# drprojects/DeepViewAgg

Measured on NVIDIA H100. Metric: Mpoints/s through view-agg fwd+bwd, higher is better.
Workload: dtype f32

## Files before the change

### deepviewagg_b200/csrc/view_attention.cuh

```cuda
#pragma once
#include "dva_common.cuh"

namespace dva {

struct VAParams {
  const void* x; const void* idx; int idx64;
  const float* compat; const int64_t* ptr;
  const float* gate_w; const float* gate_b;
  void* out; float* att; float* seg_max; float* seg_den; int32_t* seg_arg;
  const void* gout; const float* s_max; const float* s_den; const int32_t* s_arg;
  void* gx; float* gcompat; float* gate_partial; int scatter;
  int64_t N, V, R;
  int C, G, group_scaling;
  float eps;
};

constexpr int kTileStride = 33;

__device__ __forceinline__ float group_lane_sum(float v, int G) {
  for (int off = 16; off >= G; off >>= 1) v += __shfl_xor_sync(0xffffffffu, v, off);
  return v;
}

__device__ __forceinline__ uint32_t smem_u32(const void* p) { return (uint32_t)__cvta_generic_to_shared(p); }
__device__ __forceinline__ void mbar_init(uint32_t bar, uint32_t count) {
  asm volatile("mbarrier.init.shared::cta.b64 [%0], %1;" ::"r"(bar), "r"(count) : "memory");
}
__device__ __forceinline__ void mbar_init_fence() { asm volatile("fence.mbarrier_init.release.cluster;" ::: "memory"); }
__device__ __forceinline__ void mbar_expect_tx(uint32_t bar, uint32_t bytes) {
  asm volatile("mbarrier.arrive.expect_tx.shared::cta.b64 _, [%0], %1;" ::"r"(bar), "r"(bytes) : "memory");
}
__device__ __forceinline__ void mbar_wait(uint32_t bar, uint32_t parity) {
  uint32_t ok = 0;
  while (!ok) {
    asm volatile(
        "{ .reg .pred p; mbarrier.try_wait.parity.shared::cta.b64 p, [%1], %2; selp.u32 %0, 1, 0, p; }"
        : "=r"(ok) : "r"(bar), "r"(parity) : "memory");
  }
}
__device__ __forceinline__ void bulk_g2s(uint32_t dst, const void* src, uint32_t bytes, uint32_t bar) {
  asm volatile("cp.async.bulk.shared::cluster.global.mbarrier::complete_tx::bytes [%0], [%1], %2, [%3];"
               ::"r"(dst), "l"(src), "r"(bytes), "r"(bar) : "memory");
}
__device__ __forceinline__ void fence_proxy_async() { asm volatile("fence.proxy.async.shared::cta;" ::: "memory"); }

__device__ __forceinline__ uint32_t load_row_id(const void* idx, int idx64, int64_t v) {
  if (idx == nullptr) return (uint32_t)v;
  return idx64 ? (uint32_t) reinterpret_cast<const int64_t*>(idx)[v]
               : (uint32_t) reinterpret_cast<const int32_t*>(idx)[v];
}
__device__ __forceinline__ float sel4(const float4& v, int g) {
  return g == 0 ? v.x : (g == 1 ? v.y : (g == 2 ? v.z : v.w));
}

__device__ __forceinline__ float gate_t(float z) { return tanhf(fmaxf(z, 0.f)); }
__device__ __forceinline__ float4 gate_z4(const float4& w, const float4& m, const float4& b) {
  return make_float4(fmaf(w.x, m.x, b.x), fmaf(w.y, m.y, b.y), fmaf(w.z, m.z, b.z), fmaf(w.w, m.w, b.w));
}
__device__ __forceinline__ float4 gate_t4(const float4& z) {
  return make_float4(gate_t(z.x), gate_t(z.y), gate_t(z.z), gate_t(z.w));
}

__device__ __forceinline__ float gate_grad(float S, float z, float t, float w, float m, bool keep, float& dw,
                                           float& db) {
  if (!(z > 0.f)) return 0.f;
  const float dLdt = (t != 0.f) ? S / t : 0.f;
  const float u = dLdt * (1.f - t * t);
  const float dq = u * w;
  if (keep) {
    dw += u * m;
    db += u;
  }
  return dq;
}
__device__ __forceinline__ float4 gate_grad4(const float4& S, const float4& z, const float4& t, const float4& w,
                                             const float4& m, bool keep, float4& dw, float4& db) {
  return make_float4(gate_grad(S.x, z.x, t.x, w.x, m.x, keep, dw.x, db.x),
                     gate_grad(S.y, z.y, t.y, w.y, m.y, keep, dw.y, db.y),
                     gate_grad(S.z, z.z, t.z, w.z, m.z, keep, dw.z, db.z),
                     gate_grad(S.w, z.w, t.w, w.w, m.w, keep, dw.w, db.w));
}

__device__ __forceinline__ float compat_grad(float a, float sv, float S, float inv_sq, bool is_arg, float dq) {
  float d = a * (sv - S) * inv_sq;
  if (is_arg) d += dq;
  return d;
}
__device__ __forceinline__ float4 compat_grad4(const float4& a, const float4& sv, const float4& S, float inv_sq,
                                               int v, const int4& arg, const float4& dq) {
  return make_float4(compat_grad(a.x, sv.x, S.x, inv_sq, v == arg.x, dq.x),
                     compat_grad(a.y, sv.y, S.y, inv_sq, v == arg.y, dq.y),
                     compat_grad(a.z, sv.z, S.z, inv_sq, v == arg.z, dq.z),
                     compat_grad(a.w, sv.w, S.w, inv_sq, v == arg.w, dq.w));
}

template <int WARPS>
__device__ __forceinline__ void store_gate_partial(float* __restrict__ partial, const float4& dw, const float4& db) {
  __shared__ float gate_s[WARPS][8];
  const int warp = threadIdx.x >> 5, lane = threadIdx.x & 31;
  float v[8] = {dw.x, dw.y, dw.z, dw.w, db.x, db.y, db.z, db.w};
#pragma unroll
  for (int q = 0; q < 8; ++q) {
#pragma unroll
    for (int o = 16; o > 0; o >>= 1) v[q] += __shfl_xor_sync(0xffffffffu, v[q], o);
  }
  if (lane == 0) {
#pragma unroll
    for (int q = 0; q < 8; ++q) gate_s[warp][q] = v[q];
  }
  __syncthreads();
  if ((int)threadIdx.x < 8) {
    float acc = 0.f;
    for (int w = 0; w < WARPS; ++w) acc += gate_s[w][threadIdx.x];
    partial[(int64_t)blockIdx.x * 8 + threadIdx.x] = acc;
  }
}

template <typename K>
int range_geometry(K kern, size_t smem, int warps_per_cta, int max_ctas_per_sm, int ranges_per_warp, int64_t N,
                   const char* what, int* grid_out, int* pr_out) {
  cudaError_t e = cudaFuncSetAttribute(kern, cudaFuncAttributeMaxDynamicSharedMemorySize, (int)smem);
  if (e != cudaSuccess) return failf((int)e, "%s: %zu bytes of shared memory: %s", what, smem, cudaGetErrorString(e));
  int occ = 0;
  if (cudaOccupancyMaxActiveBlocksPerMultiprocessor(&occ, kern, warps_per_cta * 32, smem) != cudaSuccess || occ < 1) occ = 1;
  if (occ > max_ctas_per_sm) occ = max_ctas_per_sm;
  int64_t grid = (int64_t)kNumSMs * occ;
  const int64_t slots = grid * warps_per_cta * ranges_per_warp;
  int64_t pr = (N + slots - 1) / slots;
  if (pr < 8) pr = 8;
  const int64_t n_ranges = (N + pr - 1) / pr;
  const int64_t need = (n_ranges + warps_per_cta - 1) / warps_per_cta;
  if (grid > need) grid = need;
  if (grid < 1) grid = 1;
  *grid_out = (int)grid; *pr_out = (int)pr;
  return DVA_OK;
}

int va_ring_fwd(const VAParams& P, int dtype, cudaStream_t st);
int va_ring_bwd(const VAParams& P, int dtype, int* grid_out, cudaStream_t st);
int va_lane_bwd(const VAParams& P, int dtype, int* grid_out, cudaStream_t st);

}
```

### deepviewagg_b200/csrc/view_attention_lane.cu

```cuda
#include "view_attention.cuh"

namespace dva {

constexpr int kLaneWarps = 4;
constexpr uint32_t kFull = 0xffffffffu;

struct LaneSmem {
  float wt[32][4];
  float at[32][4];
  float st[32][4];
  float Sp[32][4];
  float dq[32][4];
  uint32_t ri[32];
  uint32_t orow[32];
  uint32_t go[32];
  uint64_t bar;
  uint64_t pad;
};

template <typename T, int LPR>
__global__ void __launch_bounds__(kLaneWarps * 32, 5)
va_lane_bwd_kernel(const VAParams P, const int PR) {
  constexpr int VEC = Vec16<T>::N, RPI = 32 / LPR, CPE = LPR / 4, U = 4, RS = LPR * 16;
  extern __shared__ __align__(128) unsigned char rows_all[];
  __shared__ LaneSmem sm_all[kLaneWarps];
  const int warp = threadIdx.x >> 5, lane = threadIdx.x & 31;
  LaneSmem& sm = sm_all[warp];
  unsigned char* rows_s = rows_all + (size_t)warp * 32 * RS;
  const uint32_t rows_u = smem_u32(rows_s), bar_u = smem_u32(&sm.bar);
  uint32_t uses = 0;
  if (lane == 0) {
    mbar_init(bar_u, 1);
    mbar_init_fence();
  }
  __syncwarp();
  const int sg = lane / LPR, lir = lane % LPR, gk = lir / CPE;
  const uint32_t row_bytes = (uint32_t)P.C * sizeof(T);
  const char* __restrict__ xbase = reinterpret_cast<const char*>(P.x);
  const char* __restrict__ gob = reinterpret_cast<const char*>(P.gout) + lir * 16;
  char* __restrict__ gxb = reinterpret_cast<char*>(P.gx) + lir * 16;
  const bool gating = P.gate_w != nullptr;
  float4 gw4 = make_float4(0.f, 0.f, 0.f, 0.f), gb4 = gw4;
  if (gating) {
    gw4 = make_float4(P.gate_w[0], P.gate_w[1], P.gate_w[2], P.gate_w[3]);
    gb4 = make_float4(P.gate_b[0], P.gate_b[1], P.gate_b[2], P.gate_b[3]);
  }
  float4 dw4 = make_float4(0.f, 0.f, 0.f, 0.f), db4 = dw4;
  const bool scatter = P.scatter && P.idx != nullptr;

  auto issue_rows = [&](int nv, uint32_t rid) {
    fence_proxy_async();
    __syncwarp();
    if (lane == 0) mbar_expect_tx(bar_u, (uint32_t)nv * row_bytes);
    __syncwarp();
    if (lane < nv) bulk_g2s(rows_u + (uint32_t)lane * RS, xbase + (uint64_t)rid * row_bytes, row_bytes, bar_u);
  };
  auto wait_rows = [&]() {
    mbar_wait(bar_u, uses & 1u);
    ++uses;
  };

  auto rows_phase = [&](int nv, int64_t pg) {
    for (int u0 = 0; u0 < nv; u0 += RPI * U) {
      uint4 xr[U], gr[U];
      float w[U];
      uint32_t orow[U];
      bool ok[U];
#pragma unroll
      for (int q = 0; q < U; ++q) {
        const int u = u0 + q * RPI + sg;
        ok[q] = u < nv;
        const int uu = ok[q] ? u : 0;
        orow[q] = sm.orow[uu];
        w[q] = sm.wt[uu][gk];
        xr[q] = *reinterpret_cast<const uint4*>(rows_s + (size_t)uu * RS + lir * 16);
        gr[q] = *reinterpret_cast<const uint4*>(gob + (uint64_t)(pg + sm.go[uu]) * row_bytes);
      }
#pragma unroll
      for (int q = 0; q < U; ++q) {
        float fx[VEC], fg[VEC], dx[VEC];
        unpack16<T, VEC>(xr[q], fx);
        unpack16<T, VEC>(gr[q], fg);
        float dot = 0.f;
#pragma unroll
        for (int j = 0; j < VEC; ++j) {
          dot = fmaf(fg[j], fx[j], dot);
          dx[j] = w[q] * fg[j];
        }
        if (ok[q]) stg_stream16(gxb + (uint64_t)orow[q] * row_bytes, pack16<T, VEC>(dx));
#pragma unroll
        for (int o = 1; o < CPE; o <<= 1) dot += __shfl_xor_sync(kFull, dot, o);
        if (ok[q] && (lir & (CPE - 1)) == 0) sm.st[u0 + q * RPI + sg][gk] = dot;
      }
    }
  };

  const int64_t n_ranges = (P.N + PR - 1) / PR;
  const int64_t warps_total = (int64_t)gridDim.x * kLaneWarps;
  for (int64_t r = (int64_t)blockIdx.x * kLaneWarps + warp; r < n_ranges; r += warps_total) {
    const int64_t pa = r * PR;
    const int64_t pb = (pa + PR < P.N) ? pa + PR : P.N;
    for (int64_t pg = pa; pg < pb;) {
      const int64_t pk = pg + lane;
      const bool valid = pk < pb;
      const int64_t p0 = valid ? P.ptr[pk] : 0;
      const int cnt = valid ? (int)(P.ptr[pk + 1] - p0) : 0;
      int incl = cnt;
#pragma unroll
      for (int o = 1; o < 32; o <<= 1) {
        const int t = __shfl_up_sync(kFull, incl, o);
        if (lane >= o) incl += t;
      }
      const int excl = incl - cnt;
      const unsigned fitm = __ballot_sync(kFull, valid && incl <= 32);
      const int kfit = (fitm == kFull) ? 32 : __ffs(~fitm) - 1;
      const int64_t gvb = __shfl_sync(kFull, p0, 0);

      if (kfit == 0) {
        const int n = __shfl_sync(kFull, cnt, 0);
        const float4 smx = reinterpret_cast<const float4*>(P.s_max)[pg];
        const float4 sdn = reinterpret_cast<const float4*>(P.s_den)[pg];
        const int4 sar = reinterpret_cast<const int4*>(P.s_arg)[pg];
        const float inv_sq = P.group_scaling ? rsqrtf((float)n) : 1.f;
        float4 z4 = make_float4(1.f, 1.f, 1.f, 1.f), t4 = z4;
        if (gating) {
          z4 = gate_z4(gw4, smx, gb4);
          t4 = gate_t4(z4);
        }
        float4 Sacc = make_float4(0.f, 0.f, 0.f, 0.f);
        for (int c0 = 0; c0 < n; c0 += 32) {
          const int nv = (n - c0 < 32) ? n - c0 : 32;
          const int64_t v = gvb + c0 + lane;
          float4 a = make_float4(0.f, 0.f, 0.f, 0.f);
          __syncwarp();
          const uint32_t rid_l = lane < nv ? load_row_id(P.idx, P.idx64, v) : 0u;
          issue_rows(nv, rid_l);
          if (lane < nv) {
            const float4 c = __ldg(reinterpret_cast<const float4*>(P.compat) + v);
            a = make_float4(__expf((c.x - smx.x) * inv_sq) / sdn.x, __expf((c.y - smx.y) * inv_sq) / sdn.y,
                            __expf((c.z - smx.z) * inv_sq) / sdn.z, __expf((c.w - smx.w) * inv_sq) / sdn.w);
            sm.ri[lane] = rid_l;
            sm.orow[lane] = scatter ? rid_l : (uint32_t)v;
            sm.go[lane] = 0u;
            *reinterpret_cast<float4*>(sm.wt[lane]) = make_float4(a.x * t4.x, a.y * t4.y, a.z * t4.z, a.w * t4.w);
          }
          __syncwarp();
          wait_rows();
          rows_phase(nv, pg);
          __syncwarp();
          if (lane < nv) {
            const float4 raw = *reinterpret_cast<const float4*>(sm.st[lane]);
            const float4 sp = make_float4(raw.x * t4.x, raw.y * t4.y, raw.z * t4.z, raw.w * t4.w);
            Sacc.x = fmaf(a.x, sp.x, Sacc.x); Sacc.y = fmaf(a.y, sp.y, Sacc.y);
            Sacc.z = fmaf(a.z, sp.z, Sacc.z); Sacc.w = fmaf(a.w, sp.w, Sacc.w);
            reinterpret_cast<float4*>(P.gcompat)[v] = sp;
          }
        }
#pragma unroll
        for (int o = 16; o > 0; o >>= 1) {
          Sacc.x += __shfl_xor_sync(kFull, Sacc.x, o); Sacc.y += __shfl_xor_sync(kFull, Sacc.y, o);
          Sacc.z += __shfl_xor_sync(kFull, Sacc.z, o); Sacc.w += __shfl_xor_sync(kFull, Sacc.w, o);
        }
        float4 dq = make_float4(0.f, 0.f, 0.f, 0.f);
        if (gating) dq = gate_grad4(Sacc, z4, t4, gw4, smx, lane == 0, dw4, db4);
        __syncwarp();
        for (int c0 = lane; c0 < n; c0 += 32) {
          const int64_t v = gvb + c0;
          const float4 c = __ldg(reinterpret_cast<const float4*>(P.compat) + v);
          const float4 sp = __ldcg(reinterpret_cast<const float4*>(P.gcompat) + v);
          float4 d;
          d.x = __expf((c.x - smx.x) * inv_sq) / sdn.x * (sp.x - Sacc.x) * inv_sq;
          d.y = __expf((c.y - smx.y) * inv_sq) / sdn.y * (sp.y - Sacc.y) * inv_sq;
          d.z = __expf((c.z - smx.z) * inv_sq) / sdn.z * (sp.z - Sacc.z) * inv_sq;
          d.w = __expf((c.w - smx.w) * inv_sq) / sdn.w * (sp.w - Sacc.w) * inv_sq;
          if ((int)v == sar.x) d.x += dq.x;
          if ((int)v == sar.y) d.y += dq.y;
          if ((int)v == sar.z) d.z += dq.z;
          if ((int)v == sar.w) d.w += dq.w;
          reinterpret_cast<float4*>(P.gcompat)[v] = d;
        }
        pg += 1;
        continue;
      }

      const int nv = __shfl_sync(kFull, incl, kfit - 1);
      int mp = 0;
      for (int k = 0; k < kfit; ++k) {
        const int s = __shfl_sync(kFull, excl, k), c = __shfl_sync(kFull, cnt, k);
        if (lane >= s && lane < s + c) mp = k;
      }
      const int cntp = __shfl_sync(kFull, cnt, mp);
      float4 a = make_float4(0.f, 0.f, 0.f, 0.f), t4 = make_float4(1.f, 1.f, 1.f, 1.f);
      float inv_sq = 1.f;
      int4 sar = make_int4(-1, -1, -1, -1);
      const int64_t v = gvb + lane;
      __syncwarp();
      const uint32_t rid_m = lane < nv ? load_row_id(P.idx, P.idx64, v) : 0u;
      if (nv > 0) issue_rows(nv, rid_m);
      if (lane < nv) {
        const float4 c = __ldg(reinterpret_cast<const float4*>(P.compat) + v);
        const float4 smx = reinterpret_cast<const float4*>(P.s_max)[pg + mp];
        const float4 sdn = reinterpret_cast<const float4*>(P.s_den)[pg + mp];
        sar = reinterpret_cast<const int4*>(P.s_arg)[pg + mp];
        inv_sq = P.group_scaling ? rsqrtf((float)cntp) : 1.f;
        a = make_float4(__expf((c.x - smx.x) * inv_sq) / sdn.x, __expf((c.y - smx.y) * inv_sq) / sdn.y,
                        __expf((c.z - smx.z) * inv_sq) / sdn.z, __expf((c.w - smx.w) * inv_sq) / sdn.w);
        if (gating) t4 = gate_t4(gate_z4(gw4, smx, gb4));
        sm.ri[lane] = rid_m;
        sm.orow[lane] = scatter ? rid_m : (uint32_t)v;
        sm.go[lane] = (uint32_t)mp;
        *reinterpret_cast<float4*>(sm.at[lane]) = a;
        *reinterpret_cast<float4*>(sm.wt[lane]) = make_float4(a.x * t4.x, a.y * t4.y, a.z * t4.z, a.w * t4.w);
      }
      __syncwarp();

      if (nv > 0) wait_rows();
      rows_phase(nv, pg);
      __syncwarp();

      if (lane < nv) {
        float4 raw = *reinterpret_cast<const float4*>(sm.st[lane]);
        raw.x *= t4.x; raw.y *= t4.y; raw.z *= t4.z; raw.w *= t4.w;
        *reinterpret_cast<float4*>(sm.st[lane]) = raw;
      }
      __syncwarp();
      if (lane < kfit) {
        float4 S = make_float4(0.f, 0.f, 0.f, 0.f), dq = S;
        for (int j = 0; j < cnt; ++j) {
          const float4 aa = *reinterpret_cast<const float4*>(sm.at[excl + j]);
          const float4 sv = *reinterpret_cast<const float4*>(sm.st[excl + j]);
          S.x = fmaf(aa.x, sv.x, S.x); S.y = fmaf(aa.y, sv.y, S.y); S.z = fmaf(aa.z, sv.z, S.z); S.w = fmaf(aa.w, sv.w, S.w);
        }
        if (gating && cnt > 0) {
          const float4 smx = reinterpret_cast<const float4*>(P.s_max)[pk];
          const float4 z4 = gate_z4(gw4, smx, gb4);
          dq = gate_grad4(S, z4, gate_t4(z4), gw4, smx, true, dw4, db4);
        }
        *reinterpret_cast<float4*>(sm.Sp[lane]) = S;
        *reinterpret_cast<float4*>(sm.dq[lane]) = dq;
      }
      __syncwarp();
      if (lane < nv) {
        const float4 S = *reinterpret_cast<const float4*>(sm.Sp[mp]);
        const float4 dq = *reinterpret_cast<const float4*>(sm.dq[mp]);
        const float4 sv = *reinterpret_cast<const float4*>(sm.st[lane]);
        reinterpret_cast<float4*>(P.gcompat)[v] = compat_grad4(a, sv, S, inv_sq, (int)v, sar, dq);
      }
      pg += kfit;
    }
  }

  if (P.gate_partial != nullptr) store_gate_partial<kLaneWarps>(P.gate_partial, dw4, db4);
}

int va_lane_bwd(const VAParams& P, int dtype, int* grid_out, cudaStream_t st) {
  return with_dtype(dtype, [&](auto tag) {
    using T = decltype(tag);
    return with_lpr(P.C / Vec16<T>::N, [&](auto lpr) {
      constexpr int LPR = decltype(lpr)::value;
      auto kern = va_lane_bwd_kernel<T, LPR>;
      const size_t smem = (size_t)kLaneWarps * 32 * LPR * 16;
      int grid, pr;
      if (int rc = range_geometry(kern, smem, kLaneWarps, 8, 4, P.N, "va_lane_bwd", &grid, &pr)) return rc;
      kern<<<grid, kLaneWarps * 32, smem, st>>>(P, pr);
      *grid_out = grid;
      return check_launch("va_lane_bwd");
    });
  });
}

}
```

Baseline: 54.22.

## Prefetch next point group rows and bulk-store dx in lane backward kernel

Restructures the lane backward kernel so that, for LPR==32, the next group's ptr ends and x rows are loaded ahead and issued via TMA while the current group finishes. dx rows are staged in shared memory and written back with a bulk async store using an evict_first L2 hint instead of per-thread streaming stores. Segment bookkeeping is simplified by loading cumulative ends directly instead of doing a prefix scan, and single-point groups use warp-shuffle reductions and a register-held gradient row instead of shared-memory round trips. The cost is more complex synchronization (bulk wait_group before reusing the row buffer) and lower min-blocks in the launch bounds for LPR==32.

```diff
diff --git a/deepviewagg_b200/csrc/view_attention.cuh b/deepviewagg_b200/csrc/view_attention.cuh
--- a/deepviewagg_b200/csrc/view_attention.cuh
+++ b/deepviewagg_b200/csrc/view_attention.cuh
@@ -43,6 +43,15 @@
                ::"r"(dst), "l"(src), "r"(bytes), "r"(bar) : "memory");
 }
 __device__ __forceinline__ void fence_proxy_async() { asm volatile("fence.proxy.async.shared::cta;" ::: "memory"); }
+__device__ __forceinline__ void bulk_s2g_evict_first(void* dst, uint32_t src, uint32_t bytes) {
+  asm volatile(
+      "{ .reg .b64 pol; createpolicy.fractional.L2::evict_first.b64 pol, 1.0;\n"
+      "  cp.async.bulk.global.shared::cta.bulk_group.L2::cache_hint [%0], [%1], %2, pol;\n"
+      "  cp.async.bulk.commit_group; }"
+      ::"l"(dst), "r"(src), "r"(bytes) : "memory");
+}
+__device__ __forceinline__ void bulk_wait_read_all() { asm volatile("cp.async.bulk.wait_group.read 0;" ::: "memory"); }
+__device__ __forceinline__ void bulk_wait_all() { asm volatile("cp.async.bulk.wait_group 0;" ::: "memory"); }
 
 __device__ __forceinline__ uint32_t load_row_id(const void* idx, int idx64, int64_t v) {
   if (idx == nullptr) return (uint32_t)v;
diff --git a/deepviewagg_b200/csrc/view_attention_lane.cu b/deepviewagg_b200/csrc/view_attention_lane.cu
--- a/deepviewagg_b200/csrc/view_attention_lane.cu
+++ b/deepviewagg_b200/csrc/view_attention_lane.cu
@@ -4,22 +4,39 @@
 
 constexpr int kLaneWarps = 4;
 constexpr uint32_t kFull = 0xffffffffu;
+constexpr int64_t kNoPoint = INT64_MAX;
 
 struct LaneSmem {
   float wt[32][4];
   float at[32][4];
   float st[32][4];
-  float Sp[32][4];
-  float dq[32][4];
-  uint32_t ri[32];
   uint32_t orow[32];
   uint32_t go[32];
   uint64_t bar;
   uint64_t pad;
 };
 
+struct LaneGroup {
+  int kfit;
+  int nv;
+  int cnt, excl;
+};
+__device__ __forceinline__ LaneGroup lane_group(int64_t e, int64_t base, int lane) {
+  const int64_t prev = __shfl_up_sync(kFull, e, 1);
+  const int64_t b = lane == 0 ? base : prev;
+  const bool valid = e != kNoPoint;
+  const unsigned fitm = __ballot_sync(kFull, valid && e - base <= 32);
+  LaneGroup g;
+  g.kfit = (fitm == kFull) ? 32 : __ffs(~fitm) - 1;
+  g.cnt = valid ? (int)(e - b) : 0;
+  const int incl = (fitm >> lane) & 1u ? (int)(e - base) : 0;
+  g.excl = incl - g.cnt;
+  g.nv = g.kfit > 0 ? __shfl_sync(kFull, incl, g.kfit - 1) : 0;
+  return g;
+}
+
 template <typename T, int LPR>
-__global__ void __launch_bounds__(kLaneWarps * 32, 5)
+__global__ void __launch_bounds__(kLaneWarps * 32, LPR == 32 ? 3 : 5)
 va_lane_bwd_kernel(const VAParams P, const int PR) {
   constexpr int VEC = Vec16<T>::N, RPI = 32 / LPR, CPE = LPR / 4, U = 4, RS = LPR * 16;
   extern __shared__ __align__(128) unsigned char rows_all[];
@@ -47,11 +64,16 @@
   }
   float4 dw4 = make_float4(0.f, 0.f, 0.f, 0.f), db4 = dw4;
   const bool scatter = P.scatter && P.idx != nullptr;
+  constexpr bool kAhead = LPR == 32;
+  const bool bulk_dx = kAhead && !scatter;
 
   auto issue_rows = [&](int nv, uint32_t rid) {
     fence_proxy_async();
     __syncwarp();
-    if (lane == 0) mbar_expect_tx(bar_u, (uint32_t)nv * row_bytes);
+    if (lane == 0) {
+      bulk_wait_read_all();
+      mbar_expect_tx(bar_u, (uint32_t)nv * row_bytes);
+    }
     __syncwarp();
     if (lane < nv) bulk_g2s(rows_u + (uint32_t)lane * RS, xbase + (uint64_t)rid * row_bytes, row_bytes, bar_u);
   };
@@ -60,7 +82,10 @@
     ++uses;
   };
 
-  auto rows_phase = [&](int nv, int64_t pg) {
+  auto rows_phase = [&](int nv, int64_t pg, bool one_point) {
+    const bool g_reg = kAhead && one_point;
+    uint4 g1 = make_uint4(0u, 0u, 0u, 0u);
+    if (g_reg) g1 = *reinterpret_cast<const uint4*>(gob + (uint64_t)pg * row_bytes);
     for (int u0 = 0; u0 < nv; u0 += RPI * U) {
       uint4 xr[U], gr[U];
       float w[U];
@@ -74,7 +99,7 @@
         orow[q] = sm.orow[uu];
         w[q] = sm.wt[uu][gk];
         xr[q] = *reinterpret_cast<const uint4*>(rows_s + (size_t)uu * RS + lir * 16);
-        gr[q] = *reinterpret_cast<const uint4*>(gob + (uint64_t)(pg + sm.go[uu]) * row_bytes);
+        gr[q] = g_reg ? g1 : *reinterpret_cast<const uint4*>(gob + (uint64_t)(pg + sm.go[uu]) * row_bytes);
       }
 #pragma unroll
       for (int q = 0; q < U; ++q) {
@@ -87,12 +112,24 @@
           dot = fmaf(fg[j], fx[j], dot);
           dx[j] = w[q] * fg[j];
         }
-        if (ok[q]) stg_stream16(gxb + (uint64_t)orow[q] * row_bytes, pack16<T, VEC>(dx));
+        if (ok[q]) {
+          if (bulk_dx) *reinterpret_cast<uint4*>(rows_s + (size_t)(u0 + q * RPI + sg) * RS + lir * 16) = pack16<T, VEC>(dx);
+          else stg_stream16(gxb + (uint64_t)orow[q] * row_bytes, pack16<T, VEC>(dx));
+        }
 #pragma unroll
         for (int o = 1; o < CPE; o <<= 1) dot += __shfl_xor_sync(kFull, dot, o);
         if (ok[q] && (lir & (CPE - 1)) == 0) sm.st[u0 + q * RPI + sg][gk] = dot;
       }
     }
+  };
+  auto store_rows = [&](int nv, int64_t v0) {
+    if (!bulk_dx || nv == 0) return;
+    fence_proxy_async();
+    __syncwarp();
+    if (lane == 0) bulk_s2g_evict_first(reinterpret_cast<char*>(P.gx) + (uint64_t)v0 * row_bytes, rows_u, (uint32_t)nv * row_bytes);
+  };
+  auto load_ends = [&](int64_t p, int64_t pb) -> int64_t {
+    return p + lane < pb ? __ldg(P.ptr + p + lane + 1) : kNoPoint;
   };
 
   const int64_t n_ranges = (P.N + PR - 1) / PR;
@@ -100,24 +137,15 @@
   for (int64_t r = (int64_t)blockIdx.x * kLaneWarps + warp; r < n_ranges; r += warps_total) {
     const int64_t pa = r * PR;
     const int64_t pb = (pa + PR < P.N) ? pa + PR : P.N;
+    int64_t gvb = __ldg(P.ptr + pa);
+    int64_t e = load_ends(pa, pb);
+    bool issued = false;
+    uint32_t rid_m = 0u;
     for (int64_t pg = pa; pg < pb;) {
-      const int64_t pk = pg + lane;
-      const bool valid = pk < pb;
-      const int64_t p0 = valid ? P.ptr[pk] : 0;
-      const int cnt = valid ? (int)(P.ptr[pk + 1] - p0) : 0;
-      int incl = cnt;
-#pragma unroll
-      for (int o = 1; o < 32; o <<= 1) {
-        const int t = __shfl_up_sync(kFull, incl, o);
-        if (lane >= o) incl += t;
-      }
-      const int excl = incl - cnt;
-      const unsigned fitm = __ballot_sync(kFull, valid && incl <= 32);
-      const int kfit = (fitm == kFull) ? 32 : __ffs(~fitm) - 1;
-      const int64_t gvb = __shfl_sync(kFull, p0, 0);
-
-      if (kfit == 0) {
-        const int n = __shfl_sync(kFull, cnt, 0);
+      const LaneGroup g = lane_group(e, gvb, lane);
+
+      if (g.kfit == 0) {
+        const int n = __shfl_sync(kFull, g.cnt, 0);
         const float4 smx = reinterpret_cast<const float4*>(P.s_max)[pg];
         const float4 sdn = reinterpret_cast<const float4*>(P.s_den)[pg];
         const int4 sar = reinterpret_cast<const int4*>(P.s_arg)[pg];
@@ -139,14 +167,14 @@
             const float4 c = __ldg(reinterpret_cast<const float4*>(P.compat) + v);
             a = make_float4(__expf((c.x - smx.x) * inv_sq) / sdn.x, __expf((c.y - smx.y) * inv_sq) / sdn.y,
                             __expf((c.z - smx.z) * inv_sq) / sdn.z, __expf((c.w - smx.w) * inv_sq) / sdn.w);
-            sm.ri[lane] = rid_l;
             sm.orow[lane] = scatter ? rid_l : (uint32_t)v;
             sm.go[lane] = 0u;
             *reinterpret_cast<float4*>(sm.wt[lane]) = make_float4(a.x * t4.x, a.y * t4.y, a.z * t4.z, a.w * t4.w);
           }
           __syncwarp();
           wait_rows();
-          rows_phase(nv, pg);
+          rows_phase(nv, pg, true);
+          store_rows(nv, gvb + c0);
           __syncwarp();
           if (lane < nv) {
             const float4 raw = *reinterpret_cast<const float4*>(sm.st[lane]);
@@ -180,23 +208,30 @@
           reinterpret_cast<float4*>(P.gcompat)[v] = d;
         }
         pg += 1;
+        gvb += n;
+        e = load_ends(pg, pb);
+        issued = false;
         continue;
       }
 
-      const int nv = __shfl_sync(kFull, incl, kfit - 1);
+      const int nv = g.nv, kfit = g.kfit;
+      const int64_t v = gvb + lane;
+      __syncwarp();
+      if (!issued) {
+        rid_m = lane < nv ? load_row_id(P.idx, P.idx64, v) : 0u;
+        if (nv > 0) issue_rows(nv, rid_m);
+      }
+      const int64_t pn = pg + kfit, gvn = gvb + nv;
+      const int64_t e_n = kAhead ? load_ends(pn, pb) : 0;
       int mp = 0;
       for (int k = 0; k < kfit; ++k) {
-        const int s = __shfl_sync(kFull, excl, k), c = __shfl_sync(kFull, cnt, k);
+        const int s = __shfl_sync(kFull, g.excl, k), c = __shfl_sync(kFull, g.cnt, k);
         if (lane >= s && lane < s + c) mp = k;
       }
-      const int cntp = __shfl_sync(kFull, cnt, mp);
+      const int cntp = __shfl_sync(kFull, g.cnt, mp);
       float4 a = make_float4(0.f, 0.f, 0.f, 0.f), t4 = make_float4(1.f, 1.f, 1.f, 1.f);
       float inv_sq = 1.f;
       int4 sar = make_int4(-1, -1, -1, -1);
-      const int64_t v = gvb + lane;
-      __syncwarp();
-      const uint32_t rid_m = lane < nv ? load_row_id(P.idx, P.idx64, v) : 0u;
-      if (nv > 0) issue_rows(nv, rid_m);
       if (lane < nv) {
         const float4 c = __ldg(reinterpret_cast<const float4*>(P.compat) + v);
         const float4 smx = reinterpret_cast<const float4*>(P.s_max)[pg + mp];
@@ -206,50 +241,71 @@
         a = make_float4(__expf((c.x - smx.x) * inv_sq) / sdn.x, __expf((c.y - smx.y) * inv_sq) / sdn.y,
                         __expf((c.z - smx.z) * inv_sq) / sdn.z, __expf((c.w - smx.w) * inv_sq) / sdn.w);
         if (gating) t4 = gate_t4(gate_z4(gw4, smx, gb4));
-        sm.ri[lane] = rid_m;
         sm.orow[lane] = scatter ? rid_m : (uint32_t)v;
         sm.go[lane] = (uint32_t)mp;
         *reinterpret_cast<float4*>(sm.at[lane]) = a;
         *reinterpret_cast<float4*>(sm.wt[lane]) = make_float4(a.x * t4.x, a.y * t4.y, a.z * t4.z, a.w * t4.w);
       }
+      LaneGroup gn{0, 0, 0, 0};
+      if (kAhead) gn = lane_group(e_n, gvn, lane);
+      const bool ahead = gn.kfit > 0 && gn.nv > 0;
+      const uint32_t rid_n = (ahead && lane < gn.nv) ? load_row_id(P.idx, P.idx64, gvn + lane) : 0u;
       __syncwarp();
 
       if (nv > 0) wait_rows();
-      rows_phase(nv, pg);
+      rows_phase(nv, pg, kfit == 1);
+      store_rows(nv, gvb);
+      if (ahead) issue_rows(gn.nv, rid_n);
       __syncwarp();
 
+      float4 sv = make_float4(0.f, 0.f, 0.f, 0.f);
       if (lane < nv) {
-        float4 raw = *reinterpret_cast<const float4*>(sm.st[lane]);
-        raw.x *= t4.x; raw.y *= t4.y; raw.z *= t4.z; raw.w *= t4.w;
-        *reinterpret_cast<float4*>(sm.st[lane]) = raw;
-      }
-      __syncwarp();
-      if (lane < kfit) {
-        float4 S = make_float4(0.f, 0.f, 0.f, 0.f), dq = S;
-        for (int j = 0; j < cnt; ++j) {
-          const float4 aa = *reinterpret_cast<const float4*>(sm.at[excl + j]);
-          const float4 sv = *reinterpret_cast<const float4*>(sm.st[excl + j]);
-          S.x = fmaf(aa.x, sv.x, S.x); S.y = fmaf(aa.y, sv.y, S.y); S.z = fmaf(aa.z, sv.z, S.z); S.w = fmaf(aa.w, sv.w, S.w);
-        }
-        if (gating && cnt > 0) {
-          const float4 smx = reinterpret_cast<const float4*>(P.s_max)[pk];
+        sv = *reinterpret_cast<const float4*>(sm.st[lane]);
+        sv.x *= t4.x; sv.y *= t4.y; sv.z *= t4.z; sv.w *= t4.w;
+      }
+      float4 S = make_float4(0.f, 0.f, 0.f, 0.f), dq = S;
+      if (kfit == 1) {
+        S = make_float4(a.x * sv.x, a.y * sv.y, a.z * sv.z, a.w * sv.w);
+#pragma unroll
+        for (int o = 16; o > 0; o >>= 1) {
+          S.x += __shfl_xor_sync(kFull, S.x, o); S.y += __shfl_xor_sync(kFull, S.y, o);
+          S.z += __shfl_xor_sync(kFull, S.z, o); S.w += __shfl_xor_sync(kFull, S.w, o);
+        }
+        if (gating && lane < nv) {
+          const float4 smx = reinterpret_cast<const float4*>(P.s_max)[pg];
           const float4 z4 = gate_z4(gw4, smx, gb4);
-          dq = gate_grad4(S, z4, gate_t4(z4), gw4, smx, true, dw4, db4);
-        }
-        *reinterpret_cast<float4*>(sm.Sp[lane]) = S;
-        *reinterpret_cast<float4*>(sm.dq[lane]) = dq;
-      }
-      __syncwarp();
-      if (lane < nv) {
-        const float4 S = *reinterpret_cast<const float4*>(sm.Sp[mp]);
-        const float4 dq = *reinterpret_cast<const float4*>(sm.dq[mp]);
-        const float4 sv = *reinterpret_cast<const float4*>(sm.st[lane]);
-        reinterpret_cast<float4*>(P.gcompat)[v] = compat_grad4(a, sv, S, inv_sq, (int)v, sar, dq);
-      }
-      pg += kfit;
+          dq = gate_grad4(S, z4, t4, gw4, smx, lane == 0, dw4, db4);
+        }
+      } else {
+        if (lane < nv) *reinterpret_cast<float4*>(sm.st[lane]) = sv;
+        __syncwarp();
+        if (lane < kfit) {
+          for (int j = 0; j < g.cnt; ++j) {
+            const float4 aa = *reinterpret_cast<const float4*>(sm.at[g.excl + j]);
+            const float4 sj = *reinterpret_cast<const float4*>(sm.st[g.excl + j]);
+            S.x = fmaf(aa.x, sj.x, S.x); S.y = fmaf(aa.y, sj.y, S.y); S.z = fmaf(aa.z, sj.z, S.z); S.w = fmaf(aa.w, sj.w, S.w);
+          }
+          if (gating && g.cnt > 0) {
+            const float4 smx = reinterpret_cast<const float4*>(P.s_max)[pg + lane];
+            const float4 z4 = gate_z4(gw4, smx, gb4);
+            dq = gate_grad4(S, z4, gate_t4(z4), gw4, smx, true, dw4, db4);
+          }
+        }
+        S.x = __shfl_sync(kFull, S.x, mp); S.y = __shfl_sync(kFull, S.y, mp);
+        S.z = __shfl_sync(kFull, S.z, mp); S.w = __shfl_sync(kFull, S.w, mp);
+        dq.x = __shfl_sync(kFull, dq.x, mp); dq.y = __shfl_sync(kFull, dq.y, mp);
+        dq.z = __shfl_sync(kFull, dq.z, mp); dq.w = __shfl_sync(kFull, dq.w, mp);
+      }
+      if (lane < nv) reinterpret_cast<float4*>(P.gcompat)[v] = compat_grad4(a, sv, S, inv_sq, (int)v, sar, dq);
+      pg = pn;
+      gvb = gvn;
+      e = kAhead ? e_n : load_ends(pn, pb);
+      rid_m = rid_n;
+      issued = ahead;
     }
   }
 
+  if (lane == 0) bulk_wait_all();
   if (P.gate_partial != nullptr) store_gate_partial<kLaneWarps>(P.gate_partial, dw4, db4);
 }
 
```

Result: faster. 54.76, median of 6 (+1.0%).
